# Dave-he/unet-watermark

Measured on AMD Instinct MI355X. Metric: train_images_per_sec, higher is better.
Workload: dtype f32 storage and accumulation; the convolution products of the encoder and decoder layers (3x3, 7x7 stem, stride-2 and 1x1 layers: forward, data gradients, and the weight gradients of the stride-1 3x3 layers and the stem) as fp16x3 splits - every fp32 operand = two fp16 halves (22 mantissa bits), a*b; 1 GPU; Unet-resnet34 512x512 bs16/GPU train step: fwd + Dice + bwd + Adam (BASELINE.json configs[1]); global_batch=16, parallelism=dp1, grad_allreduce=none

## Files before the change

include/uwm.h:

```cpp
#ifndef UWM_H
#define UWM_H
#include <stddef.h>
#include <stdint.h>

#ifdef __cplusplus
extern "C" {
#endif

typedef struct uwm_model* uwm_handle;
typedef void* uwm_stream;

enum { UWM_ENC_RESNET18 = 18, UWM_ENC_RESNET34 = 34, UWM_ENC_RESNET50 = 50,
       UWM_ENC_EFFICIENTNET_B0 = 100, UWM_ENC_EFFICIENTNET_B1 = 101, UWM_ENC_EFFICIENTNET_B2 = 102,
       UWM_ENC_EFFICIENTNET_B3 = 103, UWM_ENC_EFFICIENTNET_B4 = 104, UWM_ENC_EFFICIENTNET_B5 = 105,
       UWM_ENC_EFFICIENTNET_B6 = 106, UWM_ENC_EFFICIENTNET_B7 = 107 };
enum { UWM_ARCH_UNET = 0, UWM_ARCH_UNETPLUSPLUS = 1 };
enum { UWM_T_F32 = 0, UWM_T_I64 = 1, UWM_T_U8 = 2, UWM_T_I32 = 3 };
enum { UWM_KIND_CONV_W = 0, UWM_KIND_BIAS = 1, UWM_KIND_BN_GAMMA = 2, UWM_KIND_BN_BETA = 3,
       UWM_KIND_BN_MEAN = 4, UWM_KIND_BN_VAR = 5 };
enum { UWM_ARENA_PARAM = 0, UWM_ARENA_BUFFER = 1 };
enum { UWM_PREC_F32 = 0, UWM_PREC_BF16X3 = 1, UWM_PREC_BF16X3_ALL = 2, UWM_PREC_F16X3 = 3, UWM_PREC_F16X3_ALL = 4,
       UWM_PREC_F16X1 = 5, UWM_PREC_F16X3_BWD2 = 6 };

typedef struct {
// ... 218 lines not shown
size_t uwm_mask_workspace_bytes(int N, int H, int W);
int    uwm_optimize_mask(const uint8_t* in, uint8_t* out, int N, int H, int W, int mask_type, long long* summary,
                         void* workspace, size_t workspace_bytes, uwm_stream stream);
int    uwm_op_morph(const uint8_t* in, uint8_t* out, int N, int H, int W, int dilate, int shape, int kw, int kh,
                    int iterations, void* workspace, size_t workspace_bytes, uwm_stream stream);
int    uwm_op_components(const uint8_t* in, int32_t* labels ,
                         int32_t* areas , int N, int H, int W,
                         void* workspace, size_t workspace_bytes, uwm_stream stream);

int  uwm_set_side_stream(uwm_handle h, int on);

int  uwm_prof_enable(int on);
int  uwm_prof_collect(double* out, int max_classes);
const char* uwm_prof_class_name(int cls);

int  uwm_debug_lookup(uwm_handle h, const char* key, long long* offset, long long* count);

typedef struct {
  const float* ptr; const float* scale; const float* shift;
  int C, H, W, up, relu;
} uwm_src;
int  uwm_op_preprocess_u8_nhwc4(const uint8_t* images, long long npix, int C, const float* mean, const float* std, float* out,
                                uwm_stream stream);
int  uwm_op_set_igemm_f16x3(int on);
int  uwm_op_conv(const uwm_src* s0, const uwm_src* s1, const float* w, int wrows, int Kpad, int kh, int kw, int stride,
                 int pad, int N, int Cout, const float* bias, float* y, double* stats, int cfg, uwm_stream stream);
int  uwm_op_dgrad(const float* dy, int N, int Ho, int Wo, int Cout, const float* wd, int Cin, int KpadD, int kh, int kw,
                  int stride, int pad, int H, int W, const float* addend, const float* mask, const float* mscale,
                  const float* mshift, float* dx, uwm_stream stream);
int  uwm_op_wgrad(const uwm_src* s0, const uwm_src* s1, const float* dy, int N, int Ho, int Wo, int Cout, int wrows,
                  int Kpad, int kh, int kw, int stride, int pad, float* dw, int force_igemm, uwm_stream stream);
int  uwm_op_pack_dgrad(const float* w, int Cout, int Kpad, int ntaps, int Cin, float* wd, int KpadD, int CoutP,
                       uwm_stream stream);
int  uwm_op_maxpool(const uwm_src* in, int N, float* out, uint8_t* idx, uwm_stream stream);
int  uwm_op_maxpool_backward(const float* gout, const uint8_t* idx, const float* addend, const uwm_src* in, int N,
                             float* gin, uwm_stream stream);
int  uwm_op_bn_backward(const float* g, const float* y, const float* mean, const float* rstd, const float* gamma,
                        double* scratch2c, float* dy, float* dgamma, float* dbeta, long long npix, int C, uwm_stream stream);
int  uwm_op_bn_backward_act(const float* g, const float* y, const float* mean, const float* rstd, const float* gamma,
                            const float* scale, const float* shift, const float* se_s, const float* gpool, int N, long long hw,
                            int C, double* scratch2c, float* dy, float* dgamma, float* dbeta, float* xmax, uwm_stream stream);
int  uwm_op_dgrad_upsplit(const float* dy, int N, int H, int W, int Cout, const float* wd, int C0, int C1, int KpadD,
                          float* gprev, const float* pmask, const float* pscale, const float* pshift, float* gskip,
                          uwm_stream stream);
int  uwm_op_upsplit(const float* dcat, int N, int H, int W, int C0, int C1, float* gprev, const float* pmask,
                    const float* pscale, const float* pshift, float* gskip, uwm_stream stream);
int  uwm_op_residual(const float* y, const float* s2, const float* b2, const float* id, const float* sd, const float* bd,
                     float* out, long long npix, int C, uwm_stream stream);

#ifdef __cplusplus
}
#endif
#endif
```

unet-watermark_amd/_lib.py:

```python
from __future__ import annotations

import ctypes as C
import os
import subprocess
import sys
from pathlib import Path

os.environ.setdefault("GPU_MAX_HW_QUEUES", "8")

_PKG_DIR = Path(__file__).resolve().parent
_CSRC = _PKG_DIR / "csrc"
LIB_PATH = _PKG_DIR / "libuwm.so"
SOURCES = ["uwm_route.hip", "conv_igemm.hip", "conv_patch.hip", "conv_patch16.hip", "conv_wino.hip", "conv_wino8.hip", "conv_wino_x3.hip", "conv_f16x3.hip", "conv_f16x3v2.hip", "conv_stem_f16x3.hip", "conv_up2.hip", "conv_up2_f16.hip", "conv_c16_f16.hip", "conv_gemm.hip", "conv_head.hip", "mbconv.hip", "wgrad_igemm.hip", "wgrad_patch.hip", "wgrad_wino.hip", "wgrad_f16x3.hip", "wgrad_c16.hip", "wgrad_gemm.hip", "wgrad_stem.hip", "elementwise.hip", "loss.hip", "mask_post.hip", "resize_u8.hip", "pair_mask_u8.hip", "synth_u8.hip", "filter_u8.hip", "augment_u8.hip", "augment_ext_u8.hip", "jpeg_u8.hip", "uwm_model.hip"]
HIP_ARCH = "gfx950"
EXTRA_FLAGS = {name: ["-Xclang", "-target-feature", "-Xclang", "-packed-fp32-ops"]
               for name in ("conv_f16x3.hip", "conv_f16x3v2.hip", "wgrad_f16x3.hip", "conv_stem_f16x3.hip")}
EXTRA_FLAGS["synth_u8.hip"] = ["-ffp-contract=off"]


class uwm_unet_desc(C.Structure):
    _fields_ = [("encoder", C.c_int), ("in_channels", C.c_int), ("classes", C.c_int),
                ("decoder_channels", C.c_int * 5), ("bn_eps", C.c_float), ("bn_momentum", C.c_float), ("arch", C.c_int)]


# ... 88 lines not shown
    "uwm_op_se_scratch_floats": (L, [I, I]),
    "uwm_op_se_fc": (I, [P, P, P, I, P, P, I, I, I, I, P, P, P, P]),
    "uwm_op_se_fc_backward": (I, [P, P, P, P, P, I, P, I, I, I, I, P, P, P, P, P, P, P]),
    "uwm_op_se_scale": (I, [P, P, I, L, I, P, P]),
    "uwm_op_mb_out": (I, [P, P, P, P, P, I, L, I, P, P]),
    "uwm_op_rowscale": (I, [P, P, I, L, I, P, P]),
    "uwm_op_bn_stats": (I, [P, L, I, P, P, F, F, I, P, P, P, P, P, P, P, P]),
    "uwm_num_mbconv_blocks": (I, [P]),
    "uwm_mbconv_drop_rate": (F, [P, I]),
    "uwm_preprocess_u8": (I, [P, I, I, I, I, C.POINTER(C.c_float), C.POINTER(C.c_float), P, P, P]),
    "uwm_preprocess_mask_u8": (I, [P, I, I, I, I, P, P, P]),
    "uwm_augment_u8": (I, [P, P, P, I, I, I, I, C.POINTER(C.c_float), C.POINTER(C.c_float), I, P, P, P, P]),
    "uwm_augment_ext_workspace_bytes": (Z, [I, I, I, I]),
    "uwm_augment_ext_u8": (I, [P, P, P, P, I, I, I, I, C.POINTER(C.c_float), C.POINTER(C.c_float), I, P, Z, P, P, P, P]),
    "uwm_aug_lab_tables": (I, [I, C.POINTER(P), C.POINTER(I), C.POINTER(I)]),
    "uwm_jpeg_workspace_bytes": (Z, [I, I, I]),
    "uwm_jpeg_u8": (I, [P, P, I, I, I, C.POINTER(C.c_float), C.POINTER(C.c_float), P, Z, P, P, P]),
    "uwm_resize_threshold": (I, [P, I, I, I, I, I, I, F, I, P, P, P]),
    "uwm_mask_element": (I, [I, I, I, P]),
    "uwm_mask_workspace_bytes": (Z, [I, I, I]),
    "uwm_optimize_mask": (I, [P, P, I, I, I, I, P, P, Z, P]),
    "uwm_op_morph": (I, [P, P, I, I, I, I, I, I, I, I, P, Z, P]),
    "uwm_op_components": (I, [P, P, P, I, I, I, P, Z, P]),
    "uwm_set_side_stream": (I, [P, I]),
    "uwm_prof_enable": (I, [I]),
    "uwm_prof_collect": (I, [C.POINTER(C.c_double), I]),
    "uwm_prof_class_name": (C.c_char_p, [I]),
    "uwm_debug_lookup": (I, [P, C.c_char_p, C.POINTER(L), C.POINTER(L)]),
    "uwm_op_set_igemm_f16x3": (I, [I]),
    "uwm_op_conv": (I, [C.POINTER(uwm_src), C.POINTER(uwm_src), P, I, I, I, I, I, I, I, I, P, P, P, I, P]),
    "uwm_op_dgrad": (I, [P, I, I, I, I, P, I, I, I, I, I, I, I, I, P, P, P, P, P, P]),
    "uwm_op_wgrad": (I, [C.POINTER(uwm_src), C.POINTER(uwm_src), P, I, I, I, I, I, I, I, I, I, I, P, I, P]),
    "uwm_op_pack_dgrad": (I, [P, I, I, I, I, P, I, I, P]),
    "uwm_op_maxpool": (I, [C.POINTER(uwm_src), I, P, P, P]),
    "uwm_op_maxpool_backward": (I, [P, P, P, C.POINTER(uwm_src), I, P, P]),
    "uwm_op_bn_backward": (I, [P, P, P, P, P, P, P, P, P, L, I, P]),
    "uwm_op_bn_backward_act": (I, [P, P, P, P, P, P, P, P, P, I, L, I, P, P, P, P, P, P]),
    "uwm_op_dgrad_upsplit": (I, [P, I, I, I, I, P, I, I, I, P, P, P, P, P, P]),
    "uwm_op_upsplit": (I, [P, I, I, I, I, I, P, P, P, P, P, P]),
    "uwm_op_residual": (I, [P, P, P, P, P, P, P, L, I, P]),
}

_lib = None


def build_library(force: bool = False, verbose: bool = False) -> Path:
    srcs = [_CSRC / s for s in SOURCES]
    hdrs = [_CSRC / "uwm_kernels.h", _PKG_DIR.parent / "include" / "uwm.h"] + sorted(_CSRC.glob("*.inc"))
    if LIB_PATH.exists() and not force:
        newest = max(p.stat().st_mtime for p in srcs + hdrs)
        if LIB_PATH.stat().st_mtime >= newest:
            return LIB_PATH
    hipcc = os.environ.get("HIPCC", "/opt/rocm/bin/hipcc")
    objdir = _PKG_DIR / "build"
    objdir.mkdir(exist_ok=True)
    procs = []
    hdr_m = max(p.stat().st_mtime for p in hdrs + [Path(__file__)])
    for s in srcs:
        o = objdir / (s.stem + ".o")
        if not force and o.exists() and o.stat().st_mtime >= max(s.stat().st_mtime, hdr_m):
            procs.append((None, None, o))
            continue
        cmd = [hipcc, f"--offload-arch={HIP_ARCH}", "-O3", "-std=c++17", "-fPIC"] + EXTRA_FLAGS.get(s.name, []) + ["-c", str(s), "-o", str(o)]
        procs.append((cmd, subprocess.Popen(cmd, stdout=subprocess.PIPE, stderr=subprocess.STDOUT), o))
    objs = []
    for cmd, p, o in procs:
# ... 80 lines not shown
```

unet-watermark_amd/csrc/conv_f16x3.hip:

```cpp
#include "uwm_kernels.h"

namespace uwm {

typedef float f4 __attribute__((ext_vector_type(4)));
typedef _Float16 h8 __attribute__((ext_vector_type(8)));
typedef _Float16 h4 __attribute__((ext_vector_type(4)));

#ifndef UWM_F16_ABL
#define UWM_F16_ABL 0
#endif
constexpr int kFT = 16, kFP = kFT + 2, kFPP = kFP * kFP;
constexpr int kFPix = 40;
constexpr int kFBuf = kFPP * kFPix;
constexpr int kFKs = 5;
constexpr int kFRounds = (kFPP * 4 + 255) / 256;

__host__ __device__ inline int f16x3_nj_(int rows) { return ((rows + 63) / 64) * 4; }
int f16x3_nj(int rows) { return f16x3_nj_(rows); }
size_t f16x3_bank_floats(int rows, int chans) {
  const size_t halfs = (size_t)(chans / 16) * kFKs * f16x3_nj(rows) * 2 * 64 * 8;
  return halfs / 2 + (size_t)f16x3_nj(rows) * 16;
}
size_t f16x3_rinv_off(int rows, int chans) { return f16x3_rinv_off_floats(rows, chans); }

__device__ __forceinline__ float f16x3_wval(const WinoJob& jb, int row, int slot, int ch) {
  if (row >= jb.rows || slot >= 9 || ch >= jb.chans) return 0.f;
  if (jb.mode == 0) return jb.w[(size_t)row * jb.Kpad + (size_t)slot * jb.chans + ch];
  return ch < jb.src_rows ? jb.w[(size_t)ch * jb.Kpad + (size_t)(8 - slot) * jb.rows + row] : 0.f;
}
__global__ __launch_bounds__(256) void f16x3_rowzero_kernel(const WinoJobs jobs) {
  const WinoJob jb = jobs.j[blockIdx.y];
  if (jb.mode == 3) return;
  const int row = blockIdx.x * 256 + threadIdx.x;
  if (row < f16x3_nj_(jb.rows) * 16) (jb.ut + f16x3_rinv_off_floats(jb.rows, jb.chans))[row] = 0.f;
}
__global__ __launch_bounds__(256) void f16x3_rowmax_kernel(const WinoJobs jobs) {
  const WinoJob jb = jobs.j[blockIdx.y];
  if (jb.mode == 3) return;
  const int nJ = f16x3_nj_(jb.rows);
  unsigned* rmax = (unsigned*)(jb.ut + f16x3_rinv_off_floats(jb.rows, jb.chans));
  const int lane = threadIdx.x & 63, wv = threadIdx.x >> 6;
  const int K = 9 * jb.chans, nz = gridDim.z, z = blockIdx.z;
  if (jb.mode == 0) {
    const int row = blockIdx.x * 4 + wv;
    if (row >= jb.rows) return;
    float mx = 0.f;
    const f4* wr = (const f4*)(jb.w + (size_t)row * jb.Kpad);
    for (int i = z * 64 + lane; i < K / 4; i += nz * 64) {
      const f4 v = wr[i];
      mx = fmaxf(fmaxf(mx, fmaxf(fabsf(v.x), fabsf(v.y))), fmaxf(fabsf(v.z), fabsf(v.w)));
    }
#pragma unroll
    for (int d = 32; d >= 1; d >>= 1) mx = fmaxf(mx, __shfl_xor(mx, d));
    if (lane == 0 && mx > 0.f) atomicMax(rmax + row, __float_as_uint(mx));
  } else {
    const int row = blockIdx.x * 64 + lane;
    if (blockIdx.x * 64 >= jb.rows) return;
    float mx = 0.f;
    if (row < jb.rows)
      for (int i = z * 4 + wv; i < 9 * jb.src_rows; i += nz * 4) {
        const int ch = i / 9, tap = i - ch * 9;
        mx = fmaxf(mx, fabsf(jb.w[(size_t)ch * jb.Kpad + (size_t)tap * jb.rows + row]));
      }
    if (row < jb.rows && mx > 0.f) atomicMax(rmax + row, __float_as_uint(mx));
  }
  (void)nJ;
}
__global__ __launch_bounds__(256) void f16x3_rowscale_kernel(const WinoJobs jobs) {
  const WinoJob jb = jobs.j[blockIdx.y];
  if (jb.mode == 3) return;
  const int nJ = f16x3_nj_(jb.rows);
  const int row = blockIdx.x * 256 + threadIdx.x;
  if (row >= nJ * 16) return;
  float* rinv = jb.ut + f16x3_rinv_off_floats(jb.rows, jb.chans);
  const float mx = rinv[row];
  float s = 1.f;
  if (mx > 0.f && mx < 3.0e38f) { int e; (void)frexpf(mx, &e); s = ldexpf(1.f, 14 - e); }
  rinv[row] = 1.f / s;
}
__global__ __launch_bounds__(256) void f16x3_weights_multi_kernel(const WinoJobs jobs) {
  const WinoJob jb = jobs.j[blockIdx.y];
  if (jb.mode == 3) {
    const size_t u = blockIdx.x * (size_t)blockDim.x + threadIdx.x;
    if (u < (size_t)jb.rows * jb.Kpad / 4) ig_bank_unit(jb.w, jb.ut, u, jb.Kpad);
    return;
  }
  if (jb.pad_ == 1) return;
  const int nJ = f16x3_nj_(jb.rows);
  const size_t total = (size_t)(jb.chans / 16) * kFKs * nJ * 64;
  const size_t i = blockIdx.x * (size_t)blockDim.x + threadIdx.x;
  if (i >= total) return;
  const int lane = (int)(i & 63);
  const int j = (int)((i >> 6) % nJ);
  const int t = (int)((i >> 6) / nJ);
  const int ks = t % kFKs, chunk = t / kFKs;
  const int row = j * 16 + (lane & 15), g = lane >> 4;
  const int slot = 2 * ks + (g >> 1), ch0 = chunk * 16 + 8 * (g & 1);
  const float* rinv = jb.ut + f16x3_rinv_off_floats(jb.rows, jb.chans);
  const float s = 1.f / rinv[row];
  h8 hi, lo;
#pragma unroll
  for (int e = 0; e < 8; ++e) {
    const float v = f16x3_wval(jb, row, slot, ch0 + e) * s;
    const _Float16 h = (_Float16)v;
    hi[e] = h; lo[e] = (_Float16)(v - (float)h);
  }
  _Float16* bank = (_Float16*)jb.ut;
  h8* dst = (h8*)(bank + ((size_t)t * nJ + j) * 1024 + lane * 8);
  dst[0] = hi;
  dst[64] = lo;
}
hipError_t launch_f16x3_weights_multi(const WinoJobs& jobs, hipStream_t st) {
  if (jobs.n <= 0) return hipSuccess;
  size_t mx = 0; int mr = 0;
  for (int i = 0; i < jobs.n; ++i) {
    if (jobs.j[i].mode == 3) {
      if ((jobs.j[i].Kpad & 31) || jobs.j[i].pad_) return hipErrorInvalidValue;
      mx = std::max(mx, (size_t)jobs.j[i].rows * jobs.j[i].Kpad / 4);
      continue;
    }
    if (jobs.j[i].chans & 15) return hipErrorInvalidValue;
    const size_t t = (size_t)(jobs.j[i].chans / 16) * kFKs * f16x3_nj(jobs.j[i].rows) * 64;
    if (t > mx) mx = t;
    if (f16x3_nj(jobs.j[i].rows) * 16 > mr) mr = f16x3_nj(jobs.j[i].rows) * 16;
  }
  if (mr > 0) {
  hipLaunchKernelGGL(f16x3_rowzero_kernel, dim3((unsigned)((mr + 255) / 256), (unsigned)jobs.n), dim3(256), 0, st, jobs);
  hipLaunchKernelGGL(f16x3_rowmax_kernel, dim3((unsigned)((mr + 3) / 4), (unsigned)jobs.n, 8), dim3(256), 0, st, jobs);
  hipLaunchKernelGGL(f16x3_rowscale_kernel, dim3((unsigned)((mr + 255) / 256), (unsigned)jobs.n), dim3(256), 0, st, jobs);
  }
  hipLaunchKernelGGL(f16x3_weights_multi_kernel, dim3((unsigned)((mx + 255) / 256), (unsigned)jobs.n), dim3(256), 0, st, jobs);
  { hipError_t e = hipGetLastError(); if (e != hipSuccess) return e; }
  return launch_f16x3v2_weights_multi(jobs, st);
}

template <int NROWS>
__device__ __forceinline__ void f16x3_split_epilogue(const ConvArgs& a, const float* R, int kQLd, int row0, int n, int hb, int wb, int n0, int lane,
                                                     f4 rs, f4& ps_, f4& pq_) {
  const int cq = lane & 15, sub = lane >> 4;
  const int co = n0 + cq * 4;
  if (co >= a.Cout) return;
  if (n0 < a.up_c0) {
    const bool bnb = a.bnb_mean != nullptr;
    f4 bmu = {0.f, 0.f, 0.f, 0.f}, brs = bmu, msc = {1.f, 1.f, 1.f, 1.f}, msh = bmu;
    if (bnb) { bmu = *(const f4*)(a.bnb_mean + co); brs = *(const f4*)(a.bnb_rstd + co); }
    if (a.up_mscale) { msc = *(const f4*)(a.up_mscale + co); msh = *(const f4*)(a.up_mshift + co); }
#pragma unroll
    for (int r = 0; r < NROWS; ++r) {
      const int b = r * 4 + sub;
      const int by = b >> 3, bx = b & 7;
      const int y = row0 + 2 * by, x = 2 * bx;
      const int ho = hb + y, wo = wb + x;
      if (ho < a.Ho && wo < a.Wo) {
        const float* q = R + (y * 16 + x) * kQLd + cq * 4;
        f4 v = (*(const f4*)q + *(const f4*)(q + kQLd) + *(const f4*)(q + 16 * kQLd) + *(const f4*)(q + 17 * kQLd)) * rs;
        const size_t o2 = (((size_t)n * (a.Ho >> 1) + (ho >> 1)) * (a.Wo >> 1) + (wo >> 1)) * a.up_c0 + co;
        if (a.up_mask) {
          f4 mk = *(const f4*)(a.up_mask + o2);
          const f4 yr = mk;
          if (a.up_mscale) mk = mk * msc + msh;
          v.x = mk.x > 0.f ? v.x : 0.f; v.y = mk.y > 0.f ? v.y : 0.f;
          v.z = mk.z > 0.f ? v.z : 0.f; v.w = mk.w > 0.f ? v.w : 0.f;
          if (bnb) { ps_ += v; pq_ += v * ((yr - bmu) * brs); }
        }
// ... 583 lines not shown
```

unet-watermark_amd/csrc/elementwise.hip:

```cpp
#include "uwm_kernels.h"
#include <vector>
#include <mutex>
#include <cstdlib>

namespace uwm {

typedef float f4 __attribute__((ext_vector_type(4)));
static constexpr int kMaxBlocks = 256 * 8;

static inline unsigned nblocks(size_t work, int per_block) {
  size_t b = (work + per_block - 1) / per_block;
  if (b > (size_t)kMaxBlocks) b = kMaxBlocks;
  if (b < 1) b = 1;
  return (unsigned)b;
}

__global__ void nchw_to_nhwc4_kernel(const float* __restrict__ x, float* __restrict__ y, int C, size_t HW,
                                     size_t total, int CP) {
  for (size_t i = blockIdx.x * (size_t)blockDim.x + threadIdx.x; i < total; i += (size_t)gridDim.x * blockDim.x) {
    const size_t n = i / HW, p = i - n * HW;
    const float* xp = x + n * C * HW + p;
    float* yp = y + i * CP;
    for (int c0 = 0; c0 < CP; c0 += 4) {
      f4 v;
// ... 84 lines not shown
  hipLaunchKernelGGL(bn_eval_kernel, dim3((C + 63) / 64), dim3(64), 0, st, gamma, beta, run_mean, run_var, scale,
                     shift, C, eps);
  return hipGetLastError();
}

__global__ void residual_kernel(const float* __restrict__ y, const float* __restrict__ s2, const float* __restrict__ b2,
                                const float* __restrict__ id, const float* __restrict__ sd, const float* __restrict__ bd,
                                float* __restrict__ out, size_t n4, int C) {
  for (size_t i = blockIdx.x * (size_t)blockDim.x + threadIdx.x; i < n4; i += (size_t)gridDim.x * blockDim.x) {
    const int c = (int)((i * 4) % (size_t)C);
    f4 v = *(const f4*)(y + i * 4) * *(const f4*)(s2 + c) + *(const f4*)(b2 + c);
    f4 r = *(const f4*)(id + i * 4);
    if (sd) r = r * *(const f4*)(sd + c) + *(const f4*)(bd + c);
    v += r;
    v.x = fmaxf(v.x, 0.f); v.y = fmaxf(v.y, 0.f); v.z = fmaxf(v.z, 0.f); v.w = fmaxf(v.w, 0.f);
    *(f4*)(out + i * 4) = v;
  }
}
hipError_t launch_residual(const float* y, const float* s2, const float* b2, const float* id, const float* sd,
                           const float* bd, float* out, size_t npix, int C, hipStream_t st) {
  const size_t n4 = npix * C / 4;
  hipLaunchKernelGGL(residual_kernel, dim3(nblocks(n4, 256)), dim3(256), 0, st, y, s2, b2, id, sd, bd, out, n4, C);
  return hipGetLastError();
}

__device__ __forceinline__ f4 lazy_val(f4 v, bool has, f4 sc, f4 sh, int relu) {
  if (has) {
    v = v * sc + sh;
    if (relu) { v.x = fmaxf(v.x, 0.f); v.y = fmaxf(v.y, 0.f); v.z = fmaxf(v.z, 0.f); v.w = fmaxf(v.w, 0.f); }
  }
  return v;
}

__global__ void maxpool_fwd_kernel(const Src in, float* __restrict__ out, uint8_t* __restrict__ idx, int Ho, int Wo,
                                   size_t total) {
  const int C4 = in.C / 4;
  for (size_t i = blockIdx.x * (size_t)blockDim.x + threadIdx.x; i < total; i += (size_t)gridDim.x * blockDim.x) {
    const int c = (int)(i % C4) * 4;
    size_t p = i / C4;
    const int wo = (int)(p % Wo); p /= Wo;
    const int ho = (int)(p % Ho); const int n = (int)(p / Ho);
    const bool has = in.scale != nullptr;
    f4 sc = {1, 1, 1, 1}, sh = {0, 0, 0, 0};
    if (has) { sc = *(const f4*)(in.scale + c); sh = *(const f4*)(in.shift + c); }
    const float ninf = -__builtin_huge_valf();
    f4 best = {ninf, ninf, ninf, ninf};
    int bi[4] = {0, 0, 0, 0};
#pragma unroll
    for (int r = 0; r < 3; ++r) {
      const int h = ho * 2 - 1 + r;
      if (h < 0 || h >= in.H) continue;
#pragma unroll
      for (int s = 0; s < 3; ++s) {
        const int w = wo * 2 - 1 + s;
        if (w < 0 || w >= in.W) continue;
        f4 v = lazy_val(*(const f4*)(in.ptr + ((size_t)((size_t)n * in.H + h) * in.W + w) * in.C + c), has, sc, sh, in.relu);
        const int t = r * 3 + s;
        if (v.x > best.x) { best.x = v.x; bi[0] = t; }
        if (v.y > best.y) { best.y = v.y; bi[1] = t; }
        if (v.z > best.z) { best.z = v.z; bi[2] = t; }
        if (v.w > best.w) { best.w = v.w; bi[3] = t; }
      }
    }
    *(f4*)(out + i * 4) = best;
    if (idx) *(uchar4*)(idx + i * 4) = make_uchar4((unsigned char)bi[0], (unsigned char)bi[1], (unsigned char)bi[2], (unsigned char)bi[3]);
  }
}
hipError_t launch_maxpool_fwd(const Src& in, float* out, uint8_t* idx, int N, int Ho, int Wo, hipStream_t st) {
  const size_t total = (size_t)N * Ho * Wo * (in.C / 4);
  hipLaunchKernelGGL(maxpool_fwd_kernel, dim3(nblocks(total, 256)), dim3(256), 0, st, in, out, idx, Ho, Wo, total);
  return hipGetLastError();
}

__global__ __launch_bounds__(256) void maxpool_bwd_kernel(const float* __restrict__ gout, const uint8_t* __restrict__ idx,
                                   const float* __restrict__ addend, const Src in, float* __restrict__ gin, int Ho,
                                   int Wo, size_t total, const float* __restrict__ bn_mean, const float* __restrict__ bn_rstd,
                                   double* ssum, double* ssq, int srep, int sstride) {
  const int C4 = in.C / 4;
  f4 sg = {0.f, 0.f, 0.f, 0.f}, sgy = {0.f, 0.f, 0.f, 0.f};
  for (size_t i = blockIdx.x * (size_t)blockDim.x + threadIdx.x; i < total; i += (size_t)gridDim.x * blockDim.x) {
    const int c = (int)(i % C4) * 4;
    size_t p = i / C4;
    const int w = (int)(p % in.W); p /= in.W;
    const int h = (int)(p % in.H); const int n = (int)(p / in.H);
    f4 g = addend ? *(const f4*)(addend + i * 4) : (f4){0.f, 0.f, 0.f, 0.f};
    const int ho0 = h >> 1, ho1 = (h + 1) >> 1, wo0 = w >> 1, wo1 = (w + 1) >> 1;
    for (int a = 0; a < 2; ++a) {
      const int ho = a ? ho1 : ho0;
      if ((a && ho1 == ho0) || ho >= Ho) continue;
      const int r = h - (2 * ho - 1);
      for (int b = 0; b < 2; ++b) {
        const int wo = b ? wo1 : wo0;
        if ((b && wo1 == wo0) || wo >= Wo) continue;
        const int s = w - (2 * wo - 1);
        const size_t o = ((size_t)((size_t)n * Ho + ho) * Wo + wo) * in.C + c;
        const uchar4 id = *(const uchar4*)(idx + o);
        const f4 go = *(const f4*)(gout + o);
        const int t = r * 3 + s;
        if (id.x == t) g.x += go.x;
        if (id.y == t) g.y += go.y;
        if (id.z == t) g.z += go.z;
        if (id.w == t) g.w += go.w;
      }
// ... 642 lines not shown
```

unet-watermark_amd/csrc/loss.hip:

```cpp
#include "uwm_kernels.h"

namespace uwm {

__device__ __forceinline__ float load_target(const void* t, int dt, size_t i) {
  switch (dt) {
    case 0: return ((const float*)t)[i];
    case 1: return (float)((const long long*)t)[i];
    case 2: return (float)((const unsigned char*)t)[i];
    default: return (float)((const int*)t)[i];
  }
}

__device__ __forceinline__ double wave_sum(double v) {
#pragma unroll
  for (int d = 32; d >= 1; d >>= 1) v += __shfl_xor(v, d);
  return v;
}

__global__ __launch_bounds__(256) void loss_reduce_kernel(const float* __restrict__ logits, int ld, const void* __restrict__ target,
                                                          int tdtype, size_t n, double* scratch) {
  float s_pt = 0.f, s_p = 0.f, s_t = 0.f, s_b = 0.f;
  for (size_t i = blockIdx.x * (size_t)blockDim.x + threadIdx.x; i < n; i += (size_t)gridDim.x * blockDim.x) {
    const float x = logits[i * ld];
    const float t = load_target(target, tdtype, i);
    const float sp = log1pf(expf(-fabsf(x)));
    const float p = expf(fminf(x, 0.f) - sp);
    s_pt += p * t; s_p += p; s_t += t;
    s_b += fmaxf(x, 0.f) - x * t + sp;
  }
  __shared__ double red[4][4];
  double v0 = wave_sum((double)s_pt), v1 = wave_sum((double)s_p), v2 = wave_sum((double)s_t), v3 = wave_sum((double)s_b);
  const int wave = threadIdx.x >> 6;
  if ((threadIdx.x & 63) == 0) { red[wave][0] = v0; red[wave][1] = v1; red[wave][2] = v2; red[wave][3] = v3; }
  __syncthreads();
  if (threadIdx.x < 4) {
    const double s = red[0][threadIdx.x] + red[1][threadIdx.x] + red[2][threadIdx.x] + red[3][threadIdx.x];
    atomicAdd(scratch + threadIdx.x, s);
  }
}

struct LossCoef { double A, B; double ldice, lbce; };
__device__ __forceinline__ LossCoef loss_coef(const double* s, double n, float smooth, float eps) {
  LossCoef c;
  const double I = s[0], card = s[1] + s[2], T = s[2];
  const double den = card + (double)smooth;
  const double denc = den > (double)eps ? den : (double)eps;
  const double score = (2.0 * I + (double)smooth) / denc;
  const bool on = T > 0.0;
  c.ldice = on ? 1.0 - score : 0.0;
  c.lbce = s[3] / n;
  if (on) { c.A = 2.0 / denc; c.B = den > (double)eps ? (2.0 * I + (double)smooth) / (denc * denc) : 0.0; }
  else { c.A = 0.0; c.B = 0.0; }
  return c;
}

__global__ void loss_finalize_kernel(const double* scratch, double n, float w_dice, float w_bce, float smooth, float eps,
                                     float* out3) {
  if (threadIdx.x == 0 && blockIdx.x == 0) {
    const LossCoef c = loss_coef(scratch, n, smooth, eps);
    out3[0] = (float)((double)w_dice * c.ldice + (double)w_bce * c.lbce);
    out3[1] = (float)c.ldice;
    out3[2] = (float)c.lbce;
  }
}

__global__ __launch_bounds__(256) void loss_grad_kernel(const float* __restrict__ logits, int ld, const void* __restrict__ target,
                                                        int tdtype, size_t n, double ntotal, const double* scratch, float w_dice, float w_bce,
                                                        float smooth, float eps, float* __restrict__ dlogits, int ldd,
                                                        float gscale) {
  const LossCoef c = loss_coef(scratch, ntotal, smooth, eps);
  const float A = (float)c.A, B = (float)c.B, invn = (float)(1.0 / ntotal);
  for (size_t i = blockIdx.x * (size_t)blockDim.x + threadIdx.x; i < n; i += (size_t)gridDim.x * blockDim.x) {
    const float x = logits[i * ld];
    const float t = load_target(target, tdtype, i);
    const float sp = log1pf(expf(-fabsf(x)));
    const float p = expf(fminf(x, 0.f) - sp);
    const float gd = -(A * t - B) * p * (1.f - p);
    const float gb = (p - t) * invn;
    const float g = gscale * (w_dice * gd + w_bce * gb);
    float* o = dlogits + i * ldd;
    o[0] = g;
    for (int k = 1; k < ldd; ++k) o[k] = 0.f;
  }
}

static unsigned loss_blocks(size_t n) { size_t nb = (n + 1023) / 1024; if (nb > 2048) nb = 2048; if (nb < 1) nb = 1; return (unsigned)nb; }
hipError_t launch_loss_sums(const float* logits, int ld, const void* target, int tdtype, size_t n, double* scratch4, hipStream_t st) {
  hipError_t e = hipMemsetAsync(scratch4, 0, 4 * sizeof(double), st);
  if (e != hipSuccess) return e;
  hipLaunchKernelGGL(loss_reduce_kernel, dim3(loss_blocks(n)), dim3(256), 0, st, logits, ld, target, tdtype, n, scratch4);
  return hipGetLastError();
}
hipError_t launch_loss_apply(const float* logits, int ld, const void* target, int tdtype, size_t n, double ntotal, float w_dice, float w_bce,
                             float smooth, float eps, const double* scratch4, float* loss_out3, float* dlogits, int ldd,
                             float grad_scale, hipStream_t st) {
  hipLaunchKernelGGL(loss_finalize_kernel, dim3(1), dim3(64), 0, st, scratch4, ntotal, w_dice, w_bce, smooth, eps, loss_out3);
  if (dlogits)
    hipLaunchKernelGGL(loss_grad_kernel, dim3(loss_blocks(n)), dim3(256), 0, st, logits, ld, target, tdtype, n, ntotal, scratch4, w_dice,
                       w_bce, smooth, eps, dlogits, ldd, grad_scale);
  return hipGetLastError();
}
hipError_t launch_loss(const float* logits, int ld, const void* target, int tdtype, size_t n, float w_dice, float w_bce,
                       float smooth, float eps, double* scratch4, float* loss_out3, float* dlogits, int ldd,
                       float grad_scale, hipStream_t st) {
  hipError_t e = launch_loss_sums(logits, ld, target, tdtype, n, scratch4, st);
  if (e != hipSuccess) return e;
  return launch_loss_apply(logits, ld, target, tdtype, n, (double)n, w_dice, w_bce, smooth, eps, scratch4, loss_out3, dlogits, ldd, grad_scale, st);
}

__global__ __launch_bounds__(256) void stats_kernel(const float* __restrict__ logits, int ld, const void* __restrict__ target,
                                                    int tdtype, size_t hw, float thr, int apply_sigmoid, long long* out4) {
  const int n = blockIdx.y;
  unsigned tp = 0, po = 0, pt = 0;
  for (size_t i = blockIdx.x * (size_t)blockDim.x + threadIdx.x; i < hw; i += (size_t)gridDim.x * blockDim.x) {
    const size_t g = (size_t)n * hw + i;
    float v = logits[g * ld];
    if (apply_sigmoid) v = 1.f / (1.f + expf(-v));
    const unsigned o = v >= thr ? 1u : 0u;
    const unsigned t = load_target(target, tdtype, g) != 0.f ? 1u : 0u;
    tp += o & t; po += o; pt += t;
  }
  __shared__ unsigned red[4][3];
#pragma unroll
  for (int d = 32; d >= 1; d >>= 1) { tp += __shfl_xor(tp, d); po += __shfl_xor(po, d); pt += __shfl_xor(pt, d); }
  const int wave = threadIdx.x >> 6;
  if ((threadIdx.x & 63) == 0) { red[wave][0] = tp; red[wave][1] = po; red[wave][2] = pt; }
  __syncthreads();
  if (threadIdx.x == 0) {
    unsigned long long a = 0, b = 0, c = 0;
    for (int w = 0; w < 4; ++w) { a += red[w][0]; b += red[w][1]; c += red[w][2]; }
    unsigned long long* o = (unsigned long long*)(out4 + (size_t)n * 4);
    atomicAdd(o + 0, a);
// ... 56 lines not shown
```

unet-watermark_amd/csrc/uwm_abi.inc:

```
extern "C" {

const char* uwm_last_error(void) { return g_err; }
int uwm_version(void) { return 1; }

int uwm_create(const uwm_unet_desc* desc, uwm_handle* out) {
  if (!desc || !out) return fail("uwm_create: null argument");
  uwm_model* m = new uwm_model();
  m->desc = *desc;
  if (m->desc.bn_eps <= 0.f) m->desc.bn_eps = 1e-5f;
  if (m->desc.bn_momentum <= 0.f) m->desc.bn_momentum = 0.1f;
  if (build_model(m)) { delete m; return 1; }
  const char* e = getenv("UWM_SIDE_STREAM");
  m->use_side = e ? atoi(e) : 1;
  if (const char* pe = getenv("UWM_PRECISION")) {
    static const char* names[7] = {"f32", "bf16x3", "bf16x3_all", "f16x3", "f16x3_all", "f16x1", "f16x3_bwd2"};
    int found = -1;
    for (int i = 0; i < 7; ++i) if (!strcmp(pe, names[i]) || (pe[0] == '0' + i && !pe[1])) found = i;
    if (found < 0) { delete m; return fail("uwm_create: UWM_PRECISION=%s is not a precision mode (f32 | bf16x3 | bf16x3_all | f16x3 | f16x3_all | f16x1 | f16x3_bwd2 or 0..6)", pe); }
    m->prec = found; m->plan.prec = found; m->prec_from_env = found != UWM_PREC_F32;
  }
  if (const char* pf = getenv("UWM_F16X3_MIN_WGS")) m->f3_min_wgs = atoi(pf) > 0 ? atoi(pf) : 0;
  m->wino_mode = winograd_mode();
  m->plan.wino_mode = m->wino_mode;
  *out = m; return 0;
// ... 1059 lines not shown
}
int uwm_op_bn_backward_act(const float* g, const float* y, const float* mean, const float* rstd, const float* gamma,
                           const float* scale, const float* shift, const float* se_s, const float* gpool, int N, long long hw,
                           int C, double* scratch2c, float* dy, float* dgamma, float* dbeta, float* xmax, uwm_stream stream) {
  if (!g || !y || !mean || !rstd || !gamma || !scale || !shift || !scratch2c || !dy || !dgamma || !dbeta || N < 1 || hw < 1 ||
      C < 4 || (C & 3) || (!se_s != !gpool))
    return fail("uwm_op_bn_backward_act: bad argument");
  hipStream_t st = (hipStream_t)stream;
  HIPCHK(hipMemsetAsync(scratch2c, 0, 2 * (size_t)C * sizeof(double), st));
  if (xmax) HIPCHK(hipMemsetAsync(xmax, 0, 32 * sizeof(float), st));
  LCHK(launch_bn_bwd_act(g, y, mean, rstd, gamma, scale, shift, se_s, gpool, N, (size_t)hw, scratch2c, scratch2c + C, dy, dgamma,
                         dbeta, C, st, xmax));
  return 0;
}
int uwm_op_upsplit(const float* dcat, int N, int H, int W, int C0, int C1, float* gprev, const float* pmask,
                   const float* pscale, const float* pshift, float* gskip, uwm_stream stream) {
  if (!dcat || !gprev) return fail("uwm_op_upsplit: null argument");
  LCHK(launch_upsplit(dcat, N, H, W, C0, C1, gprev, pmask, pscale, pshift, gskip, (hipStream_t)stream));
  return 0;
}
int uwm_op_residual(const float* y, const float* s2, const float* b2, const float* id, const float* sd, const float* bd,
                    float* out, long long npix, int C, uwm_stream stream) {
  if (!y || !s2 || !b2 || !id || !out) return fail("uwm_op_residual: null argument");
  LCHK(launch_residual(y, s2, b2, id, sd, bd, out, (size_t)npix, C, (hipStream_t)stream));
  return 0;
}
int uwm_op_maxpool_backward(const float* gout, const uint8_t* idx, const float* addend, const uwm_src* in, int N, float* gin,
                            uwm_stream stream) {
  if (!gout || !idx || !in || !gin) return fail("uwm_op_maxpool_backward: null argument");
  Src s = to_src(in);
  LCHK(launch_maxpool_bwd(gout, idx, addend, s, gin, N, (s.H - 1) / 2 + 1, (s.W - 1) / 2 + 1, (hipStream_t)stream));
  return 0;
}
int uwm_op_maxpool(const uwm_src* in, int N, float* out, uint8_t* idx, uwm_stream stream) {
  if (!in || !out) return fail("uwm_op_maxpool: null argument");
  Src s = to_src(in);
  LCHK(launch_maxpool_fwd(s, out, idx, N, (s.H - 1) / 2 + 1, (s.W - 1) / 2 + 1, (hipStream_t)stream));
  return 0;
}

}
```

Before: 1180 images/s.

## Flatten f16x3 weight-prep grids, tile the maxpool forward, and fold loss finalize into grad

The f16x3 weight rowmax and pack kernels now run on a flattened 1D grid with a per-job prefix table, so each job launches only the workgroups it needs. The rowmax read is unrolled, the transposed mode uses coalesced float4 slabs, and the mode-0 pack stages through shared memory. Maxpool forward computes four outputs per thread so neighbouring windows share their loaded columns. The loss finalize kernel is merged into the gradient kernel, saving a launch. A standalone bank-packing API is added as well; the rewritten paths carry extra validation and shared-memory reduction logic that could hide bugs.

```diff
diff --git a/include/uwm.h b/include/uwm.h
--- a/include/uwm.h
+++ b/include/uwm.h
@@ -274,6 +274,9 @@
                   int Kpad, int kh, int kw, int stride, int pad, float* dw, int force_igemm, uwm_stream stream);
 int  uwm_op_pack_dgrad(const float* w, int Cout, int Kpad, int ntaps, int Cin, float* wd, int KpadD, int CoutP,
                        uwm_stream stream);
+long long uwm_op_f16x3_bank_floats(int rows, int chans);
+int  uwm_op_f16x3_bank(const float* w, int rows, int chans, int Kpad, int src_rows, int from_forward, float* bank,
+                       uwm_stream stream);
 int  uwm_op_maxpool(const uwm_src* in, int N, float* out, uint8_t* idx, uwm_stream stream);
 int  uwm_op_maxpool_backward(const float* gout, const uint8_t* idx, const float* addend, const uwm_src* in, int N,
                              float* gin, uwm_stream stream);
diff --git a/unet-watermark_amd/_lib.py b/unet-watermark_amd/_lib.py
--- a/unet-watermark_amd/_lib.py
+++ b/unet-watermark_amd/_lib.py
@@ -144,6 +144,8 @@
     "uwm_op_dgrad": (I, [P, I, I, I, I, P, I, I, I, I, I, I, I, I, P, P, P, P, P, P]),
     "uwm_op_wgrad": (I, [C.POINTER(uwm_src), C.POINTER(uwm_src), P, I, I, I, I, I, I, I, I, I, I, P, I, P]),
     "uwm_op_pack_dgrad": (I, [P, I, I, I, I, P, I, I, P]),
+    "uwm_op_f16x3_bank_floats": (L, [I, I]),
+    "uwm_op_f16x3_bank": (I, [P, I, I, I, I, I, P, P]),
     "uwm_op_maxpool": (I, [C.POINTER(uwm_src), I, P, P, P]),
     "uwm_op_maxpool_backward": (I, [P, P, P, C.POINTER(uwm_src), I, P, P]),
     "uwm_op_bn_backward": (I, [P, P, P, P, P, P, P, P, P, L, I, P]),
diff --git a/unet-watermark_amd/csrc/conv_f16x3.hip b/unet-watermark_amd/csrc/conv_f16x3.hip
--- a/unet-watermark_amd/csrc/conv_f16x3.hip
+++ b/unet-watermark_amd/csrc/conv_f16x3.hip
@@ -28,43 +28,101 @@
   if (jb.mode == 0) return jb.w[(size_t)row * jb.Kpad + (size_t)slot * jb.chans + ch];
   return ch < jb.src_rows ? jb.w[(size_t)ch * jb.Kpad + (size_t)(8 - slot) * jb.rows + row] : 0.f;
 }
+struct F16x3Grid { int first[WinoJobs::kMax + 1]; };
+static_assert(WinoJobs::kMax + 1 <= 64, "one lane per table entry");
+__device__ __forceinline__ int f16x3_grid_job(const F16x3Grid& g, int wg, int* local, int* nwg) {
+  const int lane = threadIdx.x & 63;
+  const int f = g.first[lane <= WinoJobs::kMax ? lane : WinoJobs::kMax];
+  const int j = __builtin_amdgcn_readfirstlane(__popcll(__ballot(lane <= WinoJobs::kMax && wg >= f)) - 1);
+  const int start = __builtin_amdgcn_readfirstlane(__shfl(f, j)), next = __builtin_amdgcn_readfirstlane(__shfl(f, j + 1));
+  *local = wg - start; *nwg = next - start;
+  return j;
+}
+__host__ __device__ inline int f16x3_rowmax_z(int chans) { const int z = (9 * chans / 4) / 256; return z < 1 ? 1 : (z > 8 ? 8 : z); }
+constexpr int kFMaxSlabBytes = 32768, kFMaxSlabs = 64;
+static int f16x3_rowmax_wgs(const WinoJob& jb) {
+  if (jb.mode == 3) return 0;
+  if (jb.mode == 0) return ((jb.rows + 3) / 4) * f16x3_rowmax_z(jb.chans);
+  const int pairs = jb.src_rows * 9;
+  const size_t bytes = (size_t)pairs * jb.rows * sizeof(float);
+  int n = (int)std::min<size_t>((bytes + kFMaxSlabBytes - 1) / kFMaxSlabBytes, (size_t)kFMaxSlabs);
+  n = std::max(1, std::min(n, pairs));
+  const int per = (pairs + n - 1) / n;
+  return (pairs + per - 1) / per;
+}
 __global__ __launch_bounds__(256) void f16x3_rowzero_kernel(const WinoJobs jobs) {
   const WinoJob jb = jobs.j[blockIdx.y];
   if (jb.mode == 3) return;
   const int row = blockIdx.x * 256 + threadIdx.x;
   if (row < f16x3_nj_(jb.rows) * 16) (jb.ut + f16x3_rinv_off_floats(jb.rows, jb.chans))[row] = 0.f;
 }
-__global__ __launch_bounds__(256) void f16x3_rowmax_kernel(const WinoJobs jobs) {
-  const WinoJob jb = jobs.j[blockIdx.y];
+__device__ __forceinline__ f4 f16x3_absmax4(f4 m, f4 v) {
+  return (f4){fmaxf(m.x, fabsf(v.x)), fmaxf(m.y, fabsf(v.y)), fmaxf(m.z, fabsf(v.z)), fmaxf(m.w, fabsf(v.w))};
+}
+__global__ __launch_bounds__(256) void f16x3_rowmax_kernel(const WinoJobs jobs, const F16x3Grid grid) {
+  int wg, nwg;
+  const WinoJob jb = jobs.j[f16x3_grid_job(grid, (int)blockIdx.x, &wg, &nwg)];
   if (jb.mode == 3) return;
-  const int nJ = f16x3_nj_(jb.rows);
   unsigned* rmax = (unsigned*)(jb.ut + f16x3_rinv_off_floats(jb.rows, jb.chans));
-  const int lane = threadIdx.x & 63, wv = threadIdx.x >> 6;
-  const int K = 9 * jb.chans, nz = gridDim.z, z = blockIdx.z;
+  const int tid = threadIdx.x, lane = tid & 63, wv = tid >> 6;
   if (jb.mode == 0) {
-    const int row = blockIdx.x * 4 + wv;
+    const int K = 9 * jb.chans, nbx = (jb.rows + 3) / 4, z = wg / nbx, nz = f16x3_rowmax_z(jb.chans);
+    const int row = (wg - z * nbx) * 4 + wv;
     if (row >= jb.rows) return;
     float mx = 0.f;
     const f4* wr = (const f4*)(jb.w + (size_t)row * jb.Kpad);
-    for (int i = z * 64 + lane; i < K / 4; i += nz * 64) {
-      const f4 v = wr[i];
-      mx = fmaxf(fmaxf(mx, fmaxf(fabsf(v.x), fabsf(v.y))), fmaxf(fabsf(v.z), fabsf(v.w)));
-    }
+    const int n4 = K / 4, st4 = nz * 64;
+    f4 m4 = {0.f, 0.f, 0.f, 0.f};
+    int i = z * 64 + lane;
+    for (; i + 3 * st4 < n4; i += 4 * st4) {
+      const f4 v0 = wr[i], v1 = wr[i + st4], v2 = wr[i + 2 * st4], v3 = wr[i + 3 * st4];
+      m4 = f16x3_absmax4(f16x3_absmax4(m4, v0), v1);
+      m4 = f16x3_absmax4(f16x3_absmax4(m4, v2), v3);
+    }
+    for (; i < n4; i += st4) m4 = f16x3_absmax4(m4, wr[i]);
+    mx = fmaxf(fmaxf(m4.x, m4.y), fmaxf(m4.z, m4.w));
 #pragma unroll
     for (int d = 32; d >= 1; d >>= 1) mx = fmaxf(mx, __shfl_xor(mx, d));
     if (lane == 0 && mx > 0.f) atomicMax(rmax + row, __float_as_uint(mx));
-  } else {
-    const int row = blockIdx.x * 64 + lane;
-    if (blockIdx.x * 64 >= jb.rows) return;
-    float mx = 0.f;
-    if (row < jb.rows)
-      for (int i = z * 4 + wv; i < 9 * jb.src_rows; i += nz * 4) {
-        const int ch = i / 9, tap = i - ch * 9;
-        mx = fmaxf(mx, fabsf(jb.w[(size_t)ch * jb.Kpad + (size_t)tap * jb.rows + row]));
-      }
-    if (row < jb.rows && mx > 0.f) atomicMax(rmax + row, __float_as_uint(mx));
-  }
-  (void)nJ;
+    return;
+  }
+  __shared__ f4 red[256];
+  __shared__ float fin[1024];
+  const int Q = jb.rows >> 2, Qc = Q < 256 ? Q : 256, G = 256 / Qc;
+  const int pairs = jb.src_rows * 9, per = (pairs + nwg - 1) / nwg;
+  const int p0 = wg * per, p1 = min(p0 + per, pairs);
+  const int qx = tid % Qc, g = tid / Qc;
+  for (int q = qx; q < Q; q += Qc) {
+    f4 mx = {0.f, 0.f, 0.f, 0.f};
+    if (g < G) {
+      const float* wq = jb.w + q * 4;
+      auto run = [&](int p) { const int ch = p / 9, tap = p - ch * 9; return (const f4*)(wq + (size_t)ch * jb.Kpad + (size_t)tap * jb.rows); };
+      int p = p0 + g;
+      for (; p + 3 * G < p1; p += 4 * G) {
+        const f4 v0 = *run(p), v1 = *run(p + G), v2 = *run(p + 2 * G), v3 = *run(p + 3 * G);
+        mx = f16x3_absmax4(f16x3_absmax4(mx, v0), v1);
+        mx = f16x3_absmax4(f16x3_absmax4(mx, v2), v3);
+      }
+      for (; p < p1; p += G) mx = f16x3_absmax4(mx, *run(p));
+    }
+    if (G == 1) {
+      unsigned* r = rmax + q * 4;
+      if (mx.x > 0.f) atomicMax(r + 0, __float_as_uint(mx.x));
+      if (mx.y > 0.f) atomicMax(r + 1, __float_as_uint(mx.y));
+      if (mx.z > 0.f) atomicMax(r + 2, __float_as_uint(mx.z));
+      if (mx.w > 0.f) atomicMax(r + 3, __float_as_uint(mx.w));
+      continue;
+    }
+    red[tid] = mx;
+    __syncthreads();
+    if (tid < Qc) {
+      for (int k = 1; k < G; ++k) mx = f16x3_absmax4(mx, red[k * Qc + tid]);
+      *(f4*)(fin + tid * 4) = mx;
+    }
+    __syncthreads();
+    for (int c = tid; c < jb.rows; c += 256)
+      if (fin[c] > 0.f) atomicMax(rmax + c, __float_as_uint(fin[c]));
+  }
 }
 __global__ __launch_bounds__(256) void f16x3_rowscale_kernel(const WinoJobs jobs) {
   const WinoJob jb = jobs.j[blockIdx.y];
@@ -78,17 +136,59 @@
   if (mx > 0.f && mx < 3.0e38f) { int e; (void)frexpf(mx, &e); s = ldexpf(1.f, 14 - e); }
   rinv[row] = 1.f / s;
 }
-__global__ __launch_bounds__(256) void f16x3_weights_multi_kernel(const WinoJobs jobs) {
-  const WinoJob jb = jobs.j[blockIdx.y];
+constexpr int kFPackCh = 64, kFPackLd = kFPackCh + 4;
+static int f16x3_pack_wgs(const WinoJob& jb) {
+  if (jb.mode == 3) return (int)(((size_t)jb.rows * jb.Kpad / 4 + 255) / 256);
+  if (jb.pad_ == 1) return 0;
+  if (jb.mode == 0) return f16x3_nj_(jb.rows) * kFKs * ((jb.chans + kFPackCh - 1) / kFPackCh);
+  return (int)(((size_t)(jb.chans / 16) * kFKs * f16x3_nj_(jb.rows) * 64 + 255) / 256);
+}
+__global__ __launch_bounds__(256) void f16x3_weights_multi_kernel(const WinoJobs jobs, const F16x3Grid grid) {
+  int wg, nwg;
+  const WinoJob jb = jobs.j[f16x3_grid_job(grid, (int)blockIdx.x, &wg, &nwg)];
+  (void)nwg;
   if (jb.mode == 3) {
-    const size_t u = blockIdx.x * (size_t)blockDim.x + threadIdx.x;
+    const size_t u = wg * (size_t)blockDim.x + threadIdx.x;
     if (u < (size_t)jb.rows * jb.Kpad / 4) ig_bank_unit(jb.w, jb.ut, u, jb.Kpad);
     return;
   }
-  if (jb.pad_ == 1) return;
   const int nJ = f16x3_nj_(jb.rows);
+  if (jb.mode == 0) {
+    __shared__ __attribute__((aligned(16))) float T[2 * 16 * kFPackLd];
+    const int tid = threadIdx.x;
+    const int j = wg % nJ, ks = (wg / nJ) % kFKs, cg = wg / (nJ * kFKs);
+    const float* rinv = jb.ut + f16x3_rinv_off_floats(jb.rows, jb.chans);
+    {
+      const int cq = tid & 15, r = tid >> 4, row = j * 16 + r, ch = cg * kFPackCh + cq * 4;
+      const float s = 1.f / rinv[row];
+#pragma unroll
+      for (int sl = 0; sl < 2; ++sl) {
+        const int slot = 2 * ks + sl;
+        f4 v = {0.f, 0.f, 0.f, 0.f};
+        if (row < jb.rows && slot < 9 && ch < jb.chans) v = *(const f4*)(jb.w + (size_t)row * jb.Kpad + (size_t)slot * jb.chans + ch) * s;
+        *(f4*)(T + (sl * 16 + r) * kFPackLd + cq * 4) = v;
+      }
+    }
+    __syncthreads();
+    const int lane = tid & 63, cl = tid >> 6, chunk = cg * (kFPackCh / 16) + cl;
+    if (chunk * 16 >= jb.chans) return;
+    const int g = lane >> 4;
+    const float* src = T + ((g >> 1) * 16 + (lane & 15)) * kFPackLd + cl * 16 + 8 * (g & 1);
+    const f4 a = *(const f4*)src, b = *(const f4*)(src + 4);
+    const float v8[8] = {a.x, a.y, a.z, a.w, b.x, b.y, b.z, b.w};
+    h8 hi, lo;
+#pragma unroll
+    for (int e = 0; e < 8; ++e) {
+      const _Float16 h = (_Float16)v8[e];
+      hi[e] = h; lo[e] = (_Float16)(v8[e] - (float)h);
+    }
+    h8* dst = (h8*)((_Float16*)jb.ut + ((size_t)(chunk * kFKs + ks) * nJ + j) * 1024 + lane * 8);
+    dst[0] = hi;
+    dst[64] = lo;
+    return;
+  }
   const size_t total = (size_t)(jb.chans / 16) * kFKs * nJ * 64;
-  const size_t i = blockIdx.x * (size_t)blockDim.x + threadIdx.x;
+  const size_t i = wg * (size_t)blockDim.x + threadIdx.x;
   if (i >= total) return;
   const int lane = (int)(i & 63);
   const int j = (int)((i >> 6) % nJ);
@@ -112,24 +212,30 @@
 }
 hipError_t launch_f16x3_weights_multi(const WinoJobs& jobs, hipStream_t st) {
   if (jobs.n <= 0) return hipSuccess;
-  size_t mx = 0; int mr = 0;
+  if (jobs.n > WinoJobs::kMax) return hipErrorInvalidValue;
+  int mr = 0;
+  F16x3Grid gmax, gpack;
+  gmax.first[0] = gpack.first[0] = 0;
   for (int i = 0; i < jobs.n; ++i) {
-    if (jobs.j[i].mode == 3) {
-      if ((jobs.j[i].Kpad & 31) || jobs.j[i].pad_) return hipErrorInvalidValue;
-      mx = std::max(mx, (size_t)jobs.j[i].rows * jobs.j[i].Kpad / 4);
-      continue;
-    }
-    if (jobs.j[i].chans & 15) return hipErrorInvalidValue;
-    const size_t t = (size_t)(jobs.j[i].chans / 16) * kFKs * f16x3_nj(jobs.j[i].rows) * 64;
-    if (t > mx) mx = t;
-    if (f16x3_nj(jobs.j[i].rows) * 16 > mr) mr = f16x3_nj(jobs.j[i].rows) * 16;
-  }
+    const WinoJob& jb = jobs.j[i];
+    if (jb.mode == 3) {
+      if ((jb.Kpad & 31) || jb.pad_) return hipErrorInvalidValue;
+    } else {
+      if (jb.chans & 15) return hipErrorInvalidValue;
+      if (jb.mode == 2 && ((jb.rows & 3) || (jb.Kpad & 3) || ((uintptr_t)jb.w & 15))) return hipErrorInvalidValue;
+      if (f16x3_nj(jb.rows) * 16 > mr) mr = f16x3_nj(jb.rows) * 16;
+    }
+    gmax.first[i + 1] = gmax.first[i] + f16x3_rowmax_wgs(jb);
+    gpack.first[i + 1] = gpack.first[i] + f16x3_pack_wgs(jb);
+  }
+  for (int i = jobs.n + 1; i <= WinoJobs::kMax; ++i) gmax.first[i] = gpack.first[i] = 0x7fffffff;
   if (mr > 0) {
   hipLaunchKernelGGL(f16x3_rowzero_kernel, dim3((unsigned)((mr + 255) / 256), (unsigned)jobs.n), dim3(256), 0, st, jobs);
-  hipLaunchKernelGGL(f16x3_rowmax_kernel, dim3((unsigned)((mr + 3) / 4), (unsigned)jobs.n, 8), dim3(256), 0, st, jobs);
+  hipLaunchKernelGGL(f16x3_rowmax_kernel, dim3((unsigned)gmax.first[jobs.n]), dim3(256), 0, st, jobs, gmax);
   hipLaunchKernelGGL(f16x3_rowscale_kernel, dim3((unsigned)((mr + 255) / 256), (unsigned)jobs.n), dim3(256), 0, st, jobs);
   }
-  hipLaunchKernelGGL(f16x3_weights_multi_kernel, dim3((unsigned)((mx + 255) / 256), (unsigned)jobs.n), dim3(256), 0, st, jobs);
+  if (gpack.first[jobs.n] > 0)
+    hipLaunchKernelGGL(f16x3_weights_multi_kernel, dim3((unsigned)gpack.first[jobs.n]), dim3(256), 0, st, jobs, gpack);
   { hipError_t e = hipGetLastError(); if (e != hipSuccess) return e; }
   return launch_f16x3v2_weights_multi(jobs, st);
 }
diff --git a/unet-watermark_amd/csrc/elementwise.hip b/unet-watermark_amd/csrc/elementwise.hip
--- a/unet-watermark_amd/csrc/elementwise.hip
+++ b/unet-watermark_amd/csrc/elementwise.hip
@@ -140,43 +140,64 @@
   return v;
 }
 
-__global__ void maxpool_fwd_kernel(const Src in, float* __restrict__ out, uint8_t* __restrict__ idx, int Ho, int Wo,
-                                   size_t total) {
-  const int C4 = in.C / 4;
-  for (size_t i = blockIdx.x * (size_t)blockDim.x + threadIdx.x; i < total; i += (size_t)gridDim.x * blockDim.x) {
-    const int c = (int)(i % C4) * 4;
-    size_t p = i / C4;
-    const int wo = (int)(p % Wo); p /= Wo;
-    const int ho = (int)(p % Ho); const int n = (int)(p / Ho);
-    const bool has = in.scale != nullptr;
+constexpr int kPoolRun = 4, kPoolCols = 2 * kPoolRun + 1;
+__global__ __launch_bounds__(256) void maxpool_fwd_kernel(const Src in, float* __restrict__ out, uint8_t* __restrict__ idx, int Ho, int Wo,
+                                                          int runs, unsigned total) {
+  const unsigned C4 = (unsigned)in.C / 4;
+  const bool has = in.scale != nullptr;
+  const float ninf = -__builtin_huge_valf();
+  for (unsigned i = blockIdx.x * blockDim.x + threadIdx.x; i < total; i += gridDim.x * blockDim.x) {
+    unsigned p = i / C4;
+    const int c = (int)(i - p * C4) * 4;
+    const int wo0 = (int)(p % (unsigned)runs) * kPoolRun; p /= (unsigned)runs;
+    const int ho = (int)(p % (unsigned)Ho), n = (int)(p / (unsigned)Ho);
     f4 sc = {1, 1, 1, 1}, sh = {0, 0, 0, 0};
     if (has) { sc = *(const f4*)(in.scale + c); sh = *(const f4*)(in.shift + c); }
-    const float ninf = -__builtin_huge_valf();
-    f4 best = {ninf, ninf, ninf, ninf};
-    int bi[4] = {0, 0, 0, 0};
+    f4 best[kPoolRun];
+    int bi[kPoolRun][4];
+#pragma unroll
+    for (int k = 0; k < kPoolRun; ++k) { best[k] = (f4){ninf, ninf, ninf, ninf}; bi[k][0] = bi[k][1] = bi[k][2] = bi[k][3] = 0; }
+    const int wl = wo0 * 2 - 1;
 #pragma unroll
     for (int r = 0; r < 3; ++r) {
       const int h = ho * 2 - 1 + r;
-      if (h < 0 || h >= in.H) continue;
-#pragma unroll
-      for (int s = 0; s < 3; ++s) {
-        const int w = wo * 2 - 1 + s;
-        if (w < 0 || w >= in.W) continue;
-        f4 v = lazy_val(*(const f4*)(in.ptr + ((size_t)((size_t)n * in.H + h) * in.W + w) * in.C + c), has, sc, sh, in.relu);
-        const int t = r * 3 + s;
-        if (v.x > best.x) { best.x = v.x; bi[0] = t; }
-        if (v.y > best.y) { best.y = v.y; bi[1] = t; }
-        if (v.z > best.z) { best.z = v.z; bi[2] = t; }
-        if (v.w > best.w) { best.w = v.w; bi[3] = t; }
+      const bool hok = h >= 0 && h < in.H;
+      const float* row = in.ptr + ((size_t)n * in.H + min(max(h, 0), in.H - 1)) * in.W * in.C + c;
+      f4 v[kPoolCols];
+#pragma unroll
+      for (int j = 0; j < kPoolCols; ++j) v[j] = *(const f4*)(row + (size_t)min(max(wl + j, 0), in.W - 1) * in.C);
+#pragma unroll
+      for (int j = 0; j < kPoolCols; ++j) {
+        const int w = wl + j;
+        v[j] = lazy_val(v[j], has, sc, sh, in.relu);
+        if (!(hok && w >= 0 && w < in.W)) v[j] = (f4){ninf, ninf, ninf, ninf};
       }
-    }
-    *(f4*)(out + i * 4) = best;
-    if (idx) *(uchar4*)(idx + i * 4) = make_uchar4((unsigned char)bi[0], (unsigned char)bi[1], (unsigned char)bi[2], (unsigned char)bi[3]);
+#pragma unroll
+      for (int k = 0; k < kPoolRun; ++k)
+#pragma unroll
+        for (int s = 0; s < 3; ++s) {
+          const f4 u = v[2 * k + s];
+          const int t = r * 3 + s;
+          if (u.x > best[k].x) { best[k].x = u.x; bi[k][0] = t; }
+          if (u.y > best[k].y) { best[k].y = u.y; bi[k][1] = t; }
+          if (u.z > best[k].z) { best[k].z = u.z; bi[k][2] = t; }
+          if (u.w > best[k].w) { best[k].w = u.w; bi[k][3] = t; }
+        }
+    }
+    const size_t o = (((size_t)n * Ho + ho) * Wo + wo0) * in.C + c;
+#pragma unroll
+    for (int k = 0; k < kPoolRun; ++k) {
+      if (wo0 + k >= Wo) break;
+      *(f4*)(out + o + (size_t)k * in.C) = best[k];
+      if (idx) *(uchar4*)(idx + o + (size_t)k * in.C) = make_uchar4((unsigned char)bi[k][0], (unsigned char)bi[k][1], (unsigned char)bi[k][2], (unsigned char)bi[k][3]);
+    }
   }
 }
 hipError_t launch_maxpool_fwd(const Src& in, float* out, uint8_t* idx, int N, int Ho, int Wo, hipStream_t st) {
-  const size_t total = (size_t)N * Ho * Wo * (in.C / 4);
-  hipLaunchKernelGGL(maxpool_fwd_kernel, dim3(nblocks(total, 256)), dim3(256), 0, st, in, out, idx, Ho, Wo, total);
+  const int runs = (Wo + kPoolRun - 1) / kPoolRun;
+  const size_t total = (size_t)N * Ho * runs * (in.C / 4);
+  if (total > 0x7fffffffu) return hipErrorInvalidValue;
+  hipLaunchKernelGGL(maxpool_fwd_kernel, dim3(nblocks(total, 256)), dim3(256), 0, st, in, out, idx, Ho, Wo, runs, (unsigned)total);
   return hipGetLastError();
 }
 
diff --git a/unet-watermark_amd/csrc/loss.hip b/unet-watermark_amd/csrc/loss.hip
--- a/unet-watermark_amd/csrc/loss.hip
+++ b/unet-watermark_amd/csrc/loss.hip
@@ -54,21 +54,22 @@
   return c;
 }
 
+__device__ __forceinline__ void loss_write(const LossCoef& c, float w_dice, float w_bce, float* out3) {
+  out3[0] = (float)((double)w_dice * c.ldice + (double)w_bce * c.lbce);
+  out3[1] = (float)c.ldice;
+  out3[2] = (float)c.lbce;
+}
 __global__ void loss_finalize_kernel(const double* scratch, double n, float w_dice, float w_bce, float smooth, float eps,
                                      float* out3) {
-  if (threadIdx.x == 0 && blockIdx.x == 0) {
-    const LossCoef c = loss_coef(scratch, n, smooth, eps);
-    out3[0] = (float)((double)w_dice * c.ldice + (double)w_bce * c.lbce);
-    out3[1] = (float)c.ldice;
-    out3[2] = (float)c.lbce;
-  }
+  if (threadIdx.x == 0 && blockIdx.x == 0) loss_write(loss_coef(scratch, n, smooth, eps), w_dice, w_bce, out3);
 }
 
 __global__ __launch_bounds__(256) void loss_grad_kernel(const float* __restrict__ logits, int ld, const void* __restrict__ target,
                                                         int tdtype, size_t n, double ntotal, const double* scratch, float w_dice, float w_bce,
                                                         float smooth, float eps, float* __restrict__ dlogits, int ldd,
-                                                        float gscale) {
+                                                        float gscale, float* __restrict__ out3) {
   const LossCoef c = loss_coef(scratch, ntotal, smooth, eps);
+  if (out3 && blockIdx.x == 0 && threadIdx.x == 0) loss_write(c, w_dice, w_bce, out3);
   const float A = (float)c.A, B = (float)c.B, invn = (float)(1.0 / ntotal);
   for (size_t i = blockIdx.x * (size_t)blockDim.x + threadIdx.x; i < n; i += (size_t)gridDim.x * blockDim.x) {
     const float x = logits[i * ld];
@@ -94,10 +95,11 @@
 hipError_t launch_loss_apply(const float* logits, int ld, const void* target, int tdtype, size_t n, double ntotal, float w_dice, float w_bce,
                              float smooth, float eps, const double* scratch4, float* loss_out3, float* dlogits, int ldd,
                              float grad_scale, hipStream_t st) {
-  hipLaunchKernelGGL(loss_finalize_kernel, dim3(1), dim3(64), 0, st, scratch4, ntotal, w_dice, w_bce, smooth, eps, loss_out3);
   if (dlogits)
     hipLaunchKernelGGL(loss_grad_kernel, dim3(loss_blocks(n)), dim3(256), 0, st, logits, ld, target, tdtype, n, ntotal, scratch4, w_dice,
-                       w_bce, smooth, eps, dlogits, ldd, grad_scale);
+                       w_bce, smooth, eps, dlogits, ldd, grad_scale, loss_out3);
+  else
+    hipLaunchKernelGGL(loss_finalize_kernel, dim3(1), dim3(64), 0, st, scratch4, ntotal, w_dice, w_bce, smooth, eps, loss_out3);
   return hipGetLastError();
 }
 hipError_t launch_loss(const float* logits, int ld, const void* target, int tdtype, size_t n, float w_dice, float w_bce,
diff --git a/unet-watermark_amd/csrc/uwm_abi.inc b/unet-watermark_amd/csrc/uwm_abi.inc
--- a/unet-watermark_amd/csrc/uwm_abi.inc
+++ b/unet-watermark_amd/csrc/uwm_abi.inc
@@ -1115,6 +1115,20 @@
   LCHK(launch_maxpool_bwd(gout, idx, addend, s, gin, N, (s.H - 1) / 2 + 1, (s.W - 1) / 2 + 1, (hipStream_t)stream));
   return 0;
 }
+long long uwm_op_f16x3_bank_floats(int rows, int chans) {
+  return (rows < 1 || chans < 16 || (chans & 15)) ? 0 : (long long)f16x3_bank_floats(rows, chans);
+}
+int uwm_op_f16x3_bank(const float* w, int rows, int chans, int Kpad, int src_rows, int from_forward, float* bank,
+                      uwm_stream stream) {
+  if (!w || !bank || rows < 1 || chans < 16 || (chans & 15) || src_rows < 1) return fail("uwm_op_f16x3_bank: bad argument");
+  if (from_forward ? (src_rows > chans || Kpad < 9 * rows || (rows & 3)) : (src_rows != rows || Kpad < 9 * chans))
+    return fail("uwm_op_f16x3_bank: the matrix does not hold %d rows x 9 taps x %d channels", rows, chans);
+  WinoJobs jobs; memset(&jobs, 0, sizeof(jobs)); jobs.n = 1;
+  WinoJob& j = jobs.j[0];
+  j.w = w; j.ut = bank; j.rows = rows; j.chans = chans; j.Kpad = Kpad; j.mode = from_forward ? 2 : 0; j.src_rows = src_rows; j.pad_ = 0;
+  LCHK(launch_f16x3_weights_multi(jobs, (hipStream_t)stream));
+  return 0;
+}
 int uwm_op_maxpool(const uwm_src* in, int N, float* out, uint8_t* idx, uwm_stream stream) {
   if (!in || !out) return fail("uwm_op_maxpool: null argument");
   Src s = to_src(in);
```

Measured after the change: 1192 images/s, median of 6. No clear change (+1.0%).
